# yuvalH9/UMERegRobust

Hardware: AMD Instinct MI355X
Metric: registration_pairs_per_s (higher is better)
Workload: dtype f32

## Files before the change

umeregrobust_amd/csrc/match_dev.h:

```cpp
#pragma once
#include "common.h"
#include "qlayout.h"

namespace umereg {

using f32x16 = __attribute__((ext_vector_type(16))) float;
using half8 = __attribute__((ext_vector_type(8))) _Float16;
using f32x2 = __attribute__((ext_vector_type(2))) float;

constexpr int kDistWaves = 4;

constexpr int kRegionCap = 512;
constexpr int kMaxSplits = 64;
constexpr unsigned int kShareMask = 0x8000808bu;

struct MatchScratch {
    unsigned int* rowlim;
    unsigned int* cnt;
    unsigned int* cand;
    int splits;
    unsigned int share_mask;
    int force_exhaustive;
    const int* ord1;
    const int* ord2;
    unsigned long long* stats;
};

constexpr int kCoarseTA = 2;
constexpr int kCoarseRows = kCoarseTA * 8;
constexpr int kCoarseWG = kCoarseRows * kDistWaves;

constexpr int kPK = 33;
constexpr int kPWaves = 8;
constexpr int kPRows = 32;
constexpr int kPWG = kPRows * kPWaves;
constexpr int kPRegionCap = 1024;

inline size_t qa_bytes(int n1) { return align_up((size_t)n1, 128) * 128 * sizeof(float); }
inline size_t qb_bytes(int n2) { return align_up((size_t)n2, 32) * 128 * sizeof(float); }
struct CoarsePlan {
    int n_ablk, n_blocks, n_btiles, splits, tiles_per_split;
    int sub_tiles, sub_tps, sub_splits;
};
struct MatchOpts {
    int variant = 0;
    int splits = 0;
    long long share_mask = -1;
    int exhaustive = 0;
};
inline int resolve_opts(const umereg_match_opts* o, MatchOpts& m, const char* who)
{
    m = MatchOpts();
    if (!o) return UMEREG_OK;
    UMEREG_REQUIRE(o->variant == 0 || o->variant == 1, "%s: unknown matcher variant %d (0 = Q-form, 1 = P-form)", who, (int)o->variant);
    UMEREG_REQUIRE(o->splits >= 0 && o->force_exhaustive >= 0, "%s: negative matcher option", who);
    UMEREG_REQUIRE(o->share_mask <= 0xffffffffll, "%s: share_mask does not fit 32 bits", who);
    UMEREG_REQUIRE(o->reserved == 0, "%s: umereg_match_opts.reserved must be 0 (got %d)", who, (int)o->reserved);
    m.variant = o->variant;
    m.splits = o->splits;
    m.share_mask = o->share_mask;
    m.exhaustive = o->force_exhaustive ? 1 : 0;
    return UMEREG_OK;
}
inline bool use_pform(const MatchOpts& o) { return o.variant == 1; }
constexpr int kNumCU = 256;
#ifndef UMEREG_COARSE_PHASES
#define UMEREG_COARSE_PHASES 3
#endif
constexpr int kMinSplitTiles = 4;
constexpr int kLeadMinTiles = 64;

inline CoarsePlan coarse_plan(int n1, int n2, const MatchOpts& o)
{
    CoarsePlan p;
    p.n_btiles = (n2 + 31) / 32;
    int splits;
    if (use_pform(o)) {
        p.n_ablk = (n1 + kPWG - 1) / kPWG;
        p.n_blocks = p.n_ablk * kPWaves;
        splits = kNumCU / p.n_ablk;
    } else {
        p.n_ablk = (n1 + kCoarseWG - 1) / kCoarseWG;
        p.n_blocks = p.n_ablk * kDistWaves;
        splits = (2560 + p.n_ablk - 1) / p.n_ablk;
    }
    p.sub_tiles = p.sub_tps = p.sub_splits = 0;
    if (UMEREG_COARSE_PHASES >= 2 && !use_pform(o) && o.splits <= 0 && p.n_btiles >= kLeadMinTiles) {
        const int n_sub = (n2 + kSubStride - 1) / kSubStride;
        p.sub_tiles = (n_sub + 31) / 32;
        int s1 = 4 * kNumCU / p.n_ablk;
        s1 = s1 < 1 ? 1 : (s1 > 16 ? 16 : s1);
        s1 = s1 > p.sub_tiles / kMinSplitTiles ? p.sub_tiles / kMinSplitTiles : s1;
        p.sub_tps = (p.sub_tiles + s1 - 1) / s1;
        p.sub_splits = (p.sub_tiles + p.sub_tps - 1) / p.sub_tps;
        const int bulk = p.n_btiles - p.sub_tiles;
        int s2 = splits > kMaxSplits - 16 ? kMaxSplits - 16 : splits;
        s2 = s2 > bulk / kMinSplitTiles ? bulk / kMinSplitTiles : s2;
        p.tiles_per_split = (bulk + s2 - 1) / s2;
        p.splits = p.sub_splits + (bulk + p.tiles_per_split - 1) / p.tiles_per_split;
        return p;
    }
    if (o.splits > 0) splits = o.splits;
    if (splits > kMaxSplits) splits = kMaxSplits;
    if (splits > p.n_btiles) splits = p.n_btiles;
    if (splits < 1) splits = 1;
    p.tiles_per_split = (p.n_btiles + splits - 1) / splits;
    p.splits = (p.n_btiles + p.tiles_per_split - 1) / p.tiles_per_split;
    return p;
}
inline size_t region_cap(const MatchOpts& o) { return use_pform(o) ? (size_t)kPRegionCap : (size_t)kRegionCap; }
inline size_t cand_bytes(int n1, const CoarsePlan& p, const MatchOpts& o)
{
    return align_up(((size_t)n1 + (size_t)p.n_blocks * p.splits * (1 + region_cap(o))) * sizeof(unsigned int), 256);
}
inline size_t pfrag_bytes(const CoarsePlan& p, const MatchOpts& o)
{
    return use_pform(o) ? ((size_t)p.n_blocks + (size_t)p.n_btiles) * kPK * 64 * sizeof(half8) : 0;
}
#ifndef UMEREG_COARSE_STATS
#define UMEREG_COARSE_STATS 0
#endif
constexpr size_t kStatsBytes = UMEREG_COARSE_STATS ? 256 : 0;
inline size_t match_scratch_bytes(int n1, int n2, const MatchOpts& o = MatchOpts())
{
    const CoarsePlan p = coarse_plan(n1, n2, o);
    return cand_bytes(n1, p, o) + pfrag_bytes(p, o) + kStatsBytes;
}

inline int match_args(const void* Q1_rows_h, const void* Q2_cols_h, int n1, int n2, void* scratch, size_t scratch_bytes,
                      const MatchOpts& o, const char* who)
{
    UMEREG_REQUIRE(Q1_rows_h && Q2_cols_h, "%s: null basis pointer", who);
// ... 40 lines not shown
```

umeregrobust_amd/csrc/match_f16r.hip:

```cpp
#include <type_traits>

#include "common.h"
#include "match_dev.h"
#include "qlayout.h"

namespace umereg {

constexpr float kCoarseMargin = 0.03125f + 0.0009765625f;
constexpr float kCoarseTermMax = 1.00390625f;
#ifndef UMEREG_COARSE_EXIT
#define UMEREG_COARSE_EXIT 3
#endif

__device__ __forceinline__ float group32_max(float v)
{
    int x = __float_as_int(v);
    x = __float_as_int(fmaxf(__int_as_float(x), __int_as_float(__builtin_amdgcn_mov_dpp(x, 0xB1, 0xf, 0xf, true))));
    x = __float_as_int(fmaxf(__int_as_float(x), __int_as_float(__builtin_amdgcn_mov_dpp(x, 0x4E, 0xf, 0xf, true))));
    x = __float_as_int(fmaxf(__int_as_float(x), __int_as_float(__builtin_amdgcn_mov_dpp(x, 0x141, 0xf, 0xf, true))));
    x = __float_as_int(fmaxf(__int_as_float(x), __int_as_float(__builtin_amdgcn_mov_dpp(x, 0x140, 0xf, 0xf, true))));
    x = __float_as_int(fmaxf(__int_as_float(x), __int_as_float(__builtin_amdgcn_ds_swizzle(x, 0x401F))));
    return __int_as_float(x);
}

#ifndef UMEREG_COARSE_ABLATE
#define UMEREG_COARSE_ABLATE 0
#endif
#ifndef UMEREG_COARSE_TPS
#define UMEREG_COARSE_TPS 2
#endif
constexpr int kCoarseTPS = UMEREG_COARSE_TPS;

__global__ __launch_bounds__(kWave* kDistWaves, 2) void ume_coarse_h_kernel(
    const half8* __restrict__ Afrag, const half8* __restrict__ Bfrag, int n1, int n2, int n_ablk, int tile_lo, int tile_mid, int tile_hi,
    int lead_tps, int lead_splits, int tiles_per_split, int sp0, MatchScratch ms)
{
    __shared__ half8 ldsB[2][kCoarseTPS * 512];
    const int wave = __builtin_amdgcn_readfirstlane(threadIdx.x >> 6);
    const int lane = lane_id();
    const int ablk = blockIdx.x % n_ablk;
    const int spl = blockIdx.x / n_ablk;
    const int sp = sp0 + spl;
    const bool lead = spl < lead_splits;
    const int jt0 = lead ? tile_lo + spl * lead_tps : tile_mid + (spl - lead_splits) * tiles_per_split;
    const int jt1 = lead ? min(jt0 + lead_tps, tile_mid) : min(jt0 + tiles_per_split, tile_hi);
    const int h = lane >> 5;
    const int i_base = ablk * kCoarseWG + wave * kCoarseRows;

    half8 a[kCoarseTA][2];
#pragma unroll
    for (int t = 0; t < kCoarseTA; ++t)
#pragma unroll
        for (int s = 0; s < 2; ++s)
            a[t][s] = Afrag[((((size_t)(ablk * (kCoarseWG / 8) + wave * kCoarseTA + t)) * 2 + s) * 2 + 0) * 64 + lane];

    int lim[kCoarseTA][4];
    unsigned int seen[kCoarseTA][4];
#pragma unroll
    for (int t = 0; t < kCoarseTA; ++t)
#pragma unroll
        for (int g = 0; g < 4; ++g) {
            const int i = i_base + t * 8 + 2 * g + h;
            seen[t][g] = __hip_atomic_load(ms.rowlim + min(i, n1 - 1), __ATOMIC_RELAXED, __HIP_MEMORY_SCOPE_AGENT);
            lim[t][g] = i < n1 ? max(__float_as_int(1.0e-30f), (int)seen[t][g]) : __float_as_int(3.0e38f);
        }
#pragma unroll
    for (int t = 0; t < kCoarseTA; ++t)
#pragma unroll
        for (int s = 0; s < 2; ++s) asm volatile("" ::"v"(a[t][s]));

    const int blk = ablk * kDistWaves + wave;
    unsigned int* const region = ms.cand + ((size_t)blk * ms.splits + sp) * kRegionCap;
    int qn = 0;
    auto share = [&](bool reload) __attribute__((always_inline)) {
#pragma unroll
        for (int t = 0; t < kCoarseTA; ++t)
#pragma unroll
            for (int g = 0; g < 4; ++g) {
                const float v = group32_max(__int_as_float(lim[t][g]));
                const int i = i_base + t * 8 + 2 * g + h;
                if ((lane & 31) == 0 && i < n1 && __float_as_uint(v) > seen[t][g]) atomicMax(ms.rowlim + i, __float_as_uint(v));
                lim[t][g] = max(__float_as_int(v), (int)seen[t][g]);
            }
        if (reload) {
#pragma unroll
            for (int t = 0; t < kCoarseTA; ++t)
#pragma unroll
                for (int g = 0; g < 4; ++g) {
                    const int i = min(i_base + t * 8 + 2 * g + h, n1 - 1);
                    seen[t][g] = __hip_atomic_load(ms.rowlim + i, __ATOMIC_RELAXED, __HIP_MEMORY_SCOPE_AGENT);
                }
        }
    };

    half8 st[kCoarseTPS][2];
    const int c0 = threadIdx.x, c1 = 256 + threadIdx.x;
    const int src0 = ((c0 >> 6) * 2) * 64 + (c0 & 63), src1 = ((c1 >> 6) * 2) * 64 + (c1 & 63);
    auto gload = [&](int jg) __attribute__((always_inline)) {
#pragma unroll
        for (int q = 0; q < kCoarseTPS; ++q) {
            const int jt = min(jg + q, jt1 - 1);
            st[q][0] = Bfrag[(size_t)jt * 1024 + src0];
            st[q][1] = Bfrag[(size_t)jt * 1024 + src1];
        }
    };
    auto lstore = [&](int buf) __attribute__((always_inline)) {
#pragma unroll
        for (int q = 0; q < kCoarseTPS; ++q) {
            ldsB[buf][q * 512 + c0] = st[q][0];
            ldsB[buf][q * 512 + c1] = st[q][1];
        }
    };
    if (jt0 < jt1) {
        gload(jt0);
        lstore(0);
    }
    if (jt0 + kCoarseTPS < jt1) gload(jt0 + kCoarseTPS);
    __syncthreads();
    int cur = 0;
    auto share_point = [&](const int jt) __attribute__((always_inline)) {
        const int kt = jt - jt0;
        if ((ms.share_mask >> (kt < 31 ? kt : 31)) & 1u) {
            if (kt < 31 || (kt & 31) == 31) share(true);
        }
    };
#if UMEREG_COARSE_STATS
    unsigned int n_stop1 = 0, n_stop2 = 0;
#endif
    auto hopeless = [&](const float (&sc)[kCoarseTA][4], const int cols) __attribute__((always_inline)) {
        float d = sc[0][0] - __int_as_float(lim[0][0]);
#pragma unroll
        for (int t = 0; t < kCoarseTA; ++t)
#pragma unroll
            for (int g = 0; g < 4; ++g) d = fmaxf(d, sc[t][g] - __int_as_float(lim[t][g]));
        const bool stop = __builtin_amdgcn_ballot_w64(!(d < -(float)(4 - cols) * kCoarseTermMax)) == 0ull;
        return (UMEREG_COARSE_ABLATE & 16) ? true : stop;
    };
    auto filter = [&](const int jt, const float (&sc)[kCoarseTA][4]) __attribute__((always_inline)) {
        if (UMEREG_COARSE_ABLATE & 2) {
#pragma unroll
            for (int t = 0; t < kCoarseTA; ++t)
#pragma unroll
                for (int g = 0; g < 4; ++g) lim[t][g] = max(lim[t][g], __float_as_int(sc[t][g]));
            return;
        }
#pragma unroll
        for (int t = 0; t < kCoarseTA; ++t)
#pragma unroll
            for (int g = 0; g < 4; ++g) lim[t][g] = max(lim[t][g], __float_as_int(sc[t][g] - kCoarseMargin));
        share_point(jt);
        unsigned long long hit[kCoarseTA][4], any = 0;
// ... 8 lines not shown
#pragma unroll
            for (int t = 0; t < kCoarseTA; ++t)
#pragma unroll
                for (int g = 0; g < 4; ++g) lim[t][g] = __float_as_int(group32_max(__int_as_float(lim[t][g])));
            any = 0;
#pragma unroll
            for (int t = 0; t < kCoarseTA; ++t)
#pragma unroll
                for (int g = 0; g < 4; ++g) {
                    hit[t][g] = __builtin_amdgcn_ballot_w64(sc[t][g] >= __int_as_float(lim[t][g]));
                    any |= hit[t][g];
                }
        }
        if (any) {
            const unsigned int j = (unsigned int)(jt * 32 + (lane & 31));
#pragma unroll
            for (int t = 0; t < kCoarseTA; ++t)
#pragma unroll
                for (int g = 0; g < 4; ++g) {
                    const unsigned long long mask = hit[t][g];
                    if (mask) {
                        const int pos = qn + mbcnt(mask);
                        if (((mask >> lane) & 1ull) && pos < kRegionCap)
                            region[pos] = ((unsigned int)(t * 8 + 2 * g + h) << 27) | j;
                        qn += __builtin_popcountll(mask);
                    }
                }
        }
    };
    auto tile = [&](const int jt, const int q) __attribute__((always_inline)) {
        const half8* const lB = &ldsB[cur][q * 512];
        float sc[kCoarseTA][4];
        auto products = [&](const int b, f32x16 (&cc)[kCoarseTA]) __attribute__((always_inline)) {
            const half8 b0 = (UMEREG_COARSE_ABLATE & 8) ? a[0][0] : lB[(b * 2 + 0) * 64 + lane];
            const half8 b1 = (UMEREG_COARSE_ABLATE & 8) ? a[0][1] : lB[(b * 2 + 1) * 64 + lane];
            if (UMEREG_COARSE_ABLATE & 4) {
#pragma unroll
                for (int t = 0; t < kCoarseTA; ++t)
#pragma unroll
                    for (int e = 0; e < 16; ++e) cc[t][e] = (float)b0[e & 7] + (float)b1[(e + t) & 7];
            } else {
#pragma unroll
                for (int t = 0; t < kCoarseTA; ++t) cc[t] = __builtin_amdgcn_mfma_f32_32x32x16_f16(a[t][0], b0, f32x16{0}, 0, 0, 0);
#pragma unroll
                for (int t = 0; t < kCoarseTA; ++t) cc[t] = __builtin_amdgcn_mfma_f32_32x32x16_f16(a[t][1], b1, cc[t], 0, 0, 0);
            }
        };
        auto squares = [&](const int b, const f32x16 (&cc)[kCoarseTA]) __attribute__((always_inline)) {
#pragma unroll
            for (int t = 0; t < kCoarseTA; ++t)
#pragma unroll
                for (int g = 0; g < 4; ++g) {
                    if (UMEREG_COARSE_ABLATE & 1) {
                        sc[t][g] = b == 0 ? cc[t][4 * g] : sc[t][g] + cc[t][4 * g + 1];
                        continue;
                    }
                    float acc = b == 0 ? cc[t][4 * g] * cc[t][4 * g] : fmaf(cc[t][4 * g], cc[t][4 * g], sc[t][g]);
                    acc = fmaf(cc[t][4 * g + 1], cc[t][4 * g + 1], acc);
                    acc = fmaf(cc[t][4 * g + 2], cc[t][4 * g + 2], acc);
                    sc[t][g] = fmaf(cc[t][4 * g + 3], cc[t][4 * g + 3], acc);
                }
        };
        constexpr bool kTest1 = (UMEREG_COARSE_EXIT & 1) && !(UMEREG_COARSE_ABLATE & 15), kTest2 = (UMEREG_COARSE_EXIT & 2) && !(UMEREG_COARSE_ABLATE & 15);
        constexpr bool kAhead = (UMEREG_COARSE_EXIT & 4) != 0;
        f32x16 c0[kCoarseTA], c1[kCoarseTA];
        products(0, c0);
        if (kAhead || !kTest1) products(1, c1);
        squares(0, c0);
        if (kTest1 && hopeless(sc, 1)) {
#if UMEREG_COARSE_STATS
            ++n_stop1;
#endif
            share_point(jt);
            return;
        }
        if (!kAhead && kTest1) products(1, c1);
        squares(1, c1);
        if (kTest2 && hopeless(sc, 2)) {
#if UMEREG_COARSE_STATS
            ++n_stop2;
#endif
            share_point(jt);
            return;
        }
#pragma unroll
        for (int b = 2; b < 4; ++b) {
            f32x16 cc[kCoarseTA];
            products(b, cc);
            squares(b, cc);
        }
        filter(jt, sc);
    };
    for (int jg = jt0; jg < jt1; jg += kCoarseTPS) {
#pragma unroll
        for (int q = 0; q < kCoarseTPS; ++q)
            if (jg + q < jt1) tile(jg + q, q);
        if (jg + kCoarseTPS < jt1) lstore(cur ^ 1);
        if (jg + 2 * kCoarseTPS < jt1) gload(jg + 2 * kCoarseTPS);
        __syncthreads();
        cur ^= 1;
    }
    share(false);
    if (lane == 0) ms.cnt[(size_t)blk * ms.splits + sp] = (unsigned int)qn;
#if UMEREG_COARSE_STATS
    if (lane == 0) {
        atomicAdd(ms.stats + 0, (unsigned long long)max(jt1 - jt0, 0));
        atomicAdd(ms.stats + 1, (unsigned long long)n_stop1);
        atomicAdd(ms.stats + 2, (unsigned long long)n_stop2);
        atomicAdd(ms.stats + 3, (unsigned long long)qn);
    }
#endif
}

constexpr float kCoarseMarginP = 0.009765625f;
constexpr int kPDepth = 5;
constexpr int kQsStride = 33;

__global__ __launch_bounds__(256) void pform_pack_kernel(const _Float16* __restrict__ Ah, const _Float16* __restrict__ Bh, int n1,
                                                         int n2, int tiles1, int tiles2, half8* __restrict__ PA,
                                                         half8* __restrict__ PB)
{
    __shared__ float4 qs[32 * kQsStride];
    const int side = blockIdx.y, tile = blockIdx.x;
    if (tile >= (side ? tiles2 : tiles1)) return;
    const int n = side ? n2 : n1;
    const _Float16* const Q = side ? Bh : Ah;
    half8* const P = (side ? PB : PA) + (size_t)tile * kPK * 64;
    const int tid = threadIdx.x;
    if (tile * 32 >= n) {
        for (int o = tid; o < kPK * 64; o += 256) P[o] = half8{0};
        return;
// ... 396 lines not shown
```

umeregrobust_amd/csrc/ball_moment.hip:

```cpp
#include "grid.h"

namespace umereg {

constexpr int kPackWG = 1024;
constexpr int kPackMaxBlocks = 32;

__global__ __launch_bounds__(kPackWG) void pack_points_kernel(const float* __restrict__ pts, char* __restrict__ ws,
                                                              size_t ws_stride, int N, const PairDesc* __restrict__ desc)
{
    __shared__ unsigned int red[kPackWG / 64][6];
    const GridWs w = grid_ws(N);
    const int b = blockIdx.y;
    const int n_live = desc ? desc->n_pts[b] : N;
    const UMEREG_GLOBAL_AS float* __restrict__ src = global_ptr(desc ? desc->pts[b] : pts + (size_t)b * N * 3);
    float4* out = reinterpret_cast<float4*>(ws + b * ws_stride + w.off_p4o);
    unsigned int* bbox = reinterpret_cast<unsigned int*>(ws + b * ws_stride + w.off_bbox);
    unsigned int e[6] = {0u, 0u, 0u, 0u, 0u, 0u};
    for (int j = blockIdx.x * kPackWG + threadIdx.x; j < w.Npad; j += gridDim.x * kPackWG) {
        float4 v = make_float4(kFar, kFar, kFar, 0.f);
        if (j < n_live) {
            const UMEREG_GLOBAL_AS float* p = src + (size_t)j * 3;
            v = make_float4(p[0], p[1], p[2], 0.f);
            const unsigned int ex = enc_ord(v.x), ey = enc_ord(v.y), ez = enc_ord(v.z);
            e[0] = max(e[0], ~ex); e[1] = max(e[1], ~ey); e[2] = max(e[2], ~ez);
// ... 297 lines not shown
                                                const Grid& g, float qx, float qy, float qz, float r2, int K,
                                                int n_eff, int nbits, int* lst, int cap, int lane)
{
    const float rq = sqrtf(r2) * 1.0001f + 1e-20f;
    const int y0 = cell_axis(qy - rq, g.miny, g.invy, g.ny), y1 = cell_axis(qy + rq, g.miny, g.invy, g.ny);
    const int z0 = cell_axis(qz - rq, g.minz, g.invz, g.nz), z1 = cell_axis(qz + rq, g.minz, g.invz, g.nz);
    const float csy = 1.0f / g.invy, csz = 1.0f / g.invz;
    const float rq2 = rq * rq;
    int cnt = 0;
    int thr = n_eff - 1;
    const int ny_r = y1 - y0 + 1, n_rows = ny_r * (z1 - z0 + 1);
    for (int r0 = 0; r0 < n_rows; r0 += kWave) {
        int my_beg = 0, my_end = 0;
        {
            const int r = r0 + lane;
            const int z = z0 + r / ny_r, y = y0 + r % ny_r;
            const float z_a = g.minz + (float)z * csz, z_b = z_a + csz;
            const float dzc = fmaxf(fmaxf(z > 0 ? z_a - qz : 0.f, z < g.nz - 1 ? qz - z_b : 0.f), 0.f) * 0.9999f;
            const float y_a = g.miny + (float)y * csy, y_b = y_a + csy;
            const float dyc = fmaxf(fmaxf(y > 0 ? y_a - qy : 0.f, y < g.ny - 1 ? qy - y_b : 0.f), 0.f) * 0.9999f;
            const float rem = rq2 - dyc * dyc - dzc * dzc;
            if (r < n_rows && rem > 0.f) {
                const float sx = sqrtf(rem) * 1.0001f + 1e-20f;
                const int cbase = (z * g.ny + y) * g.nx;
                my_beg = start[cbase + cell_axis(qx - sx, g.minx, g.invx, g.nx)];
                my_end = start[cbase + cell_axis(qx + sx, g.minx, g.invx, g.nx) + 1];
            }
        }
        const int n_here = min(kWave, n_rows - r0);
        for (int rr = 0; rr < n_here; ++rr) {
            const int beg = __builtin_amdgcn_readlane(my_beg, rr);
            const int end = __builtin_amdgcn_readlane(my_end, rr);
            if (beg >= end) continue;
            auto scan = [&](int base, auto U_) __attribute__((always_inline)) {
                constexpr int U = decltype(U_)::value;
                float4 pv[U];
#pragma unroll
                for (int u = 0; u < U; ++u) {
                    const int pos = base + u * kWave + lane;
                    pv[u] = P4s[pos < end ? pos : end - 1];
                }
#pragma unroll
                for (int u = 0; u < U; ++u) {
                    const int pos = base + u * kWave + lane;
                    const float4 p = pv[u];
                    const int oi = __float_as_int(p.w);
                    const float dx = qx - p.x;
                    const float dy = qy - p.y;
                    const float dz = qz - p.z;
                    const float d2 = dist2_as_the_reference<kFma>(dx, dy, dz);
                    const bool hit = (pos < end) && (d2 < r2) && (oi <= thr);
                    const unsigned long long m = __ballot(hit);
                    if (m != 0ull) {
                        if (hit) lst[cnt + mbcnt(m)] = oi;
                        cnt += __popcll(m);
                    }
                }
            };
            auto make_room = [&](int chunks) __attribute__((always_inline)) {
                if (cnt > cap - chunks * kWave) {
                    __builtin_amdgcn_wave_barrier();
                    cnt = keep_k_smallest(lst, cnt, K, nbits, cap, lane, thr);
                }
            };
            int base = beg;
            for (; end - base > 2 * kWave; base += kWave * kScanUnroll) { make_room(kScanUnroll); scan(base, std::integral_constant<int, kScanUnroll>{}); }
            if (base < end) { make_room(2); scan(base, std::integral_constant<int, 2>{}); }
        }
    }
    __builtin_amdgcn_wave_barrier();
    if (cnt > K) cnt = keep_k_smallest(lst, cnt, K, nbits, cap, lane, thr);
    return cnt;
}

__device__ __forceinline__ void bitonic_sort(int* lst, int n_pow2, int lane)
{
    for (int k = 2; k <= n_pow2; k <<= 1)
        for (int j = k >> 1; j > 0; j >>= 1) {
            __builtin_amdgcn_wave_barrier();
            for (int t = lane; t < (n_pow2 >> 1); t += kWave) {
                const int lo = ((t & ~(j - 1)) << 1) | (t & (j - 1));
                const int hi = lo | j;
                const bool up = (lo & k) == 0;
                const int a = lst[lo], b = lst[hi];
                if ((a > b) == up) { lst[lo] = b; lst[hi] = a; }
            }
        }
    __builtin_amdgcn_wave_barrier();
}

__device__ __forceinline__ void sort_kept(int* lst, int count, int lane)
{
    int n_pow2 = 64;
    while (n_pow2 < count) n_pow2 <<= 1;
    for (int e = count + lane; e < n_pow2; e += kWave) lst[e] = 0x7fffffff;
    bitonic_sort(lst, n_pow2, lane);
}

template <bool kFma>
__global__ __launch_bounds__(256) void ball_query_kernel(
// ... 86 lines not shown
    for (int k = threadIdx.x + kKeep * 1024; k < n_kp; k += 1024) atomicAdd(&cnt[cell_of_kp(k)], 1);
    __syncthreads();
    const int c0 = threadIdx.x * 4;
    const int t0 = cnt[c0], t1 = cnt[c0 + 1], t2 = cnt[c0 + 2], t3 = cnt[c0 + 3];
    const int sum = t0 + t1 + t2 + t3;
    int incl = sum;
#pragma unroll
    for (int m = 1; m < 64; m <<= 1) {
        const int o = __shfl_up(incl, m, kWave);
        if ((int)(threadIdx.x & 63) >= m) incl += o;
    }
    if ((threadIdx.x & 63) == 63) part[threadIdx.x >> 6] = incl;
    __syncthreads();
    int base = 0;
    for (int k = 0; k < (int)(threadIdx.x >> 6); ++k) base += part[k];
    const int excl = base + incl - sum;
    __syncthreads();
    cnt[c0] = excl; cnt[c0 + 1] = excl + t0; cnt[c0 + 2] = excl + t0 + t1; cnt[c0 + 3] = excl + t0 + t1 + t2;
    __syncthreads();
#pragma unroll
    for (int u = 0; u < kKeep; ++u)
        if (mine[u] >= 0) perm[atomicAdd(&cnt[mine[u]], 1)] = threadIdx.x + u * 1024;
    for (int k = threadIdx.x + kKeep * 1024; k < n_kp; k += 1024) perm[atomicAdd(&cnt[cell_of_kp(k)], 1)] = k;
}

__device__ __forceinline__ float bcast8(float v)
{
    int x = __float_as_int(v);
    x = __builtin_amdgcn_mov_dpp(x, 0x00, 0xf, 0xf, true);
    x = __builtin_amdgcn_update_dpp(x, x, 0x114, 0xf, 0xa, false);
    return __int_as_float(x);
}

constexpr int kMomUnroll = 4;

template <int kAcc, bool kFma = false, bool kDesc = false>
__global__ __launch_bounds__(256) void ume_moments_kernel(
    const char* __restrict__ ws, size_t ws_stride, const float* __restrict__ kpts,
    const int64_t* __restrict__ kp_index, const float4* __restrict__ feat4, int N, int n_kp, int K, int cap,
    float radius, int flags, float* __restrict__ F, int32_t* __restrict__ nn_count,
    int64_t* __restrict__ nn_idx)
{
    const bool ordered = flags & UMEREG_MOMENTS_ORDERED;
    extern __shared__ int lds[];
    const int wave = __builtin_amdgcn_readfirstlane(threadIdx.x >> 6);
    const int lane = lane_id();
    const int b = blockIdx.y;
    const GridWs w = grid_ws(N);
    const char* wb = ws + b * ws_stride;
    int kp;
    if (ordered) {
        const int nblk = gridDim.x, xcd = blockIdx.x & 7, q = nblk >> 3, r = nblk & 7;
        const int lblk = (xcd < r ? xcd * (q + 1) : r * (q + 1) + (xcd - r) * q) + (blockIdx.x >> 3);
        const int slot = lblk * (blockDim.x >> 6) + wave;
        if (slot >= n_kp) return;
        kp = __builtin_amdgcn_readfirstlane(reinterpret_cast<const int*>(wb + w.off_kperm)[slot]);
    } else {
        kp = blockIdx.x * (blockDim.x >> 6) + wave;
        if (kp >= n_kp) return;
    }
    int* lst = lds + wave * cap;
    const float4* Pb = reinterpret_cast<const float4*>(wb + w.off_p4o);
    const float4* P4s = reinterpret_cast<const float4*>(wb + w.off_p4s);
    const int* start = reinterpret_cast<const int*>(wb + w.off_start);
    const Grid g = load_grid(reinterpret_cast<const unsigned int*>(wb + w.off_bbox), radius, N);
    const unsigned int* __restrict__ rec = reinterpret_cast<const unsigned int*>(wb + w.off_bbox);
// ... 9 lines not shown
            for (int e = lane; e < 128; e += kWave) F[((size_t)b * n_kp + kp) * 128 + e] = __int_as_float(0x7fc00000);
            if (nn_count && lane == 0) nn_count[(size_t)b * n_kp + kp] = 0;
            if (nn_idx) for (int e = lane; e < K; e += kWave) nn_idx[((size_t)b * n_kp + kp) * K + e] = -1;
            return;
        }
        const float4 qp = Pb[ki];
        qx = qp.x; qy = qp.y; qz = qp.z;
    } else {
        const float* q = kpts + ((size_t)b * n_kp + kp) * 3;
        qx = q[0]; qy = q[1]; qz = q[2];
    }
    const int nbits = 32 - __clz(N > 1 ? N - 1 : 1);

    const int count = ball_search_grid<kFma>(P4s, start, g, qx, qy, qz, radius * radius, K, n_live, nbits, lst, cap, lane);

    if (nn_count && lane == 0) nn_count[(size_t)b * n_kp + kp] = count;
    if (nn_idx) {
        sort_kept(lst, count, lane);
        int64_t* o = nn_idx + ((size_t)b * n_kp + kp) * K;
        for (int e = lane; e < K; e += kWave) o[e] = e < count ? (int64_t)lst[e] : (int64_t)-1;
    }

    constexpr bool kF64 = kAcc != 0;
#ifndef UMEREG_MOM_ABLATE
#define UMEREG_MOM_ABLATE 0
#endif
#ifndef UMEREG_MOM_MFMA_UNROLL
#define UMEREG_MOM_MFMA_UNROLL 4
#endif
    if (kAcc == 2) {
        constexpr int kMU = UMEREG_MOM_MFMA_UNROLL;
        const int mk = lane >> 4, mr = lane & 15, mcq = mr & 7, mns = 4 * (mr >> 3) + mk, mj = lane & 3;
        const float* Pf = reinterpret_cast<const float*>(Pb);
        double acc[4] = {0.0, 0.0, 0.0, 0.0};
        auto mtrip = [&](int e0, bool ragged, auto U_) __attribute__((always_inline)) {
            constexpr int kU = decltype(U_)::value;
            float4 ff[kU];
            float pc[kU];
#pragma unroll
            for (int u = 0; u < kU; ++u) {
                const unsigned int jn = (unsigned int)lst[min(e0 + u * 8 + mns, count - 1)];
                if (UMEREG_MOM_ABLATE & 2) {
                    const float v = __uint_as_float(0x3f800000u | (jn & 0xffffu));
                    ff[u] = make_float4(v, v + 1.f, v + 2.f, v + 3.f);
                    pc[u] = v;
                    continue;
                }
                ff[u] = feat_slice((size_t)jn * 8 + mcq);
                pc[u] = Pf[(size_t)jn * 4 + (mj > 0 ? mj - 1 : 0)];
            }
            if (UMEREG_MOM_ABLATE & 4) {
                float t = 0.f;
#pragma unroll
                for (int u = 0; u < kU; ++u) t += ((ff[u].x + ff[u].y) + (ff[u].z + ff[u].w)) + pc[u];
                acc[0] += (double)t;
                return;
            }
#pragma unroll
            for (int u = 0; u < kU; ++u) {
                if (ragged) {
                    const bool v = e0 + u * 8 + mns < count;
                    ff[u].x = v ? ff[u].x : 0.f; ff[u].y = v ? ff[u].y : 0.f;
                    ff[u].z = v ? ff[u].z : 0.f; ff[u].w = v ? ff[u].w : 0.f;
                }
                const double bq = mj == 0 ? 1.0 : (double)pc[u];
                acc[0] = __builtin_amdgcn_mfma_f64_4x4x4f64((double)ff[u].x, bq, acc[0], 0, 0, 0);
                acc[1] = __builtin_amdgcn_mfma_f64_4x4x4f64((double)ff[u].y, bq, acc[1], 0, 0, 0);
                acc[2] = __builtin_amdgcn_mfma_f64_4x4x4f64((double)ff[u].z, bq, acc[2], 0, 0, 0);
                acc[3] = __builtin_amdgcn_mfma_f64_4x4x4f64((double)ff[u].w, bq, acc[3], 0, 0, 0);
            }
        };
#ifndef UMEREG_MOM_PIPE
#define UMEREG_MOM_PIPE 0
#endif
#if UMEREG_MOM_PIPE
        constexpr int kH = kMU / 2 > 0 ? kMU / 2 : 1;
        auto load_half = [&](int e0, float4 (&ff)[kH], float (&pc)[kH]) __attribute__((always_inline)) {
#pragma unroll
            for (int u = 0; u < kH; ++u) {
                if (e0 + u * 8 < count) {
                    const unsigned int jn = (unsigned int)lst[min(e0 + u * 8 + mns, count - 1)];
                    ff[u] = feat_slice((size_t)jn * 8 + mcq);
                    pc[u] = Pf[(size_t)jn * 4 + (mj > 0 ? mj - 1 : 0)];
                }
            }
        };
        auto fma_half = [&](int e0, float4 (&ff)[kH], float (&pc)[kH]) __attribute__((always_inline)) {
#pragma unroll
            for (int u = 0; u < kH; ++u) {
                if (e0 + u * 8 < count) {
                    if (e0 + u * 8 + 8 > count) {
                        const bool v = e0 + u * 8 + mns < count;
                        ff[u].x = v ? ff[u].x : 0.f; ff[u].y = v ? ff[u].y : 0.f;
                        ff[u].z = v ? ff[u].z : 0.f; ff[u].w = v ? ff[u].w : 0.f;
                    }
                    const double bq = mj == 0 ? 1.0 : (double)pc[u];
                    acc[0] = __builtin_amdgcn_mfma_f64_4x4x4f64((double)ff[u].x, bq, acc[0], 0, 0, 0);
                    acc[1] = __builtin_amdgcn_mfma_f64_4x4x4f64((double)ff[u].y, bq, acc[1], 0, 0, 0);
                    acc[2] = __builtin_amdgcn_mfma_f64_4x4x4f64((double)ff[u].z, bq, acc[2], 0, 0, 0);
                    acc[3] = __builtin_amdgcn_mfma_f64_4x4x4f64((double)ff[u].w, bq, acc[3], 0, 0, 0);
                }
            }
        };
        {
            float4 fa[kH], fc[kH];
            float pa[kH], pq[kH];
            const int step = 8 * kH;
            const int n_half = (UMEREG_MOM_ABLATE & 1) ? 0 : (count + step - 1) / step;
            if (n_half > 0) load_half(0, fa, pa);
            for (int h = 0; h < n_half; h += 2) {
                if (h + 1 < n_half) load_half((h + 1) * step, fc, pq);
                fma_half(h * step, fa, pa);
                if (h + 2 < n_half) load_half((h + 2) * step, fa, pa);
                if (h + 1 < n_half) fma_half((h + 1) * step, fc, pq);
            }
        }
        (void)mtrip;
#else
        const int mfull = (UMEREG_MOM_ABLATE & 1) ? 0 : (count / (8 * kMU)) * (8 * kMU);
        for (int e0 = 0; e0 < mfull; e0 += 8 * kMU) mtrip(e0, false, std::integral_constant<int, kMU>{});
        if (!(UMEREG_MOM_ABLATE & 1))
        for (int e0 = mfull; e0 < count; e0 += 8) mtrip(e0, e0 + 8 > count, std::integral_constant<int, 1>{});
#endif
#pragma unroll
        for (int m = 0; m < 4; ++m) acc[m] += shfl_xor_f64(acc[m], 8);
        const bool lower = (lane & 8) == 0;
        double s = (lower && mj == 0) ? (acc[0] + acc[1]) + (acc[2] + acc[3]) : 0.0;
#pragma unroll
        for (int m = 1; m < 64; m <<= 1) s += shfl_xor_f64(s, m);
// ... 217 lines not shown
    UMEREG_REQUIRE(pts && packed, "pack_points: null pointer");
    UMEREG_REQUIRE(B > 0 && N > 0, "pack_points: B, N must be positive (got %d, %d)", B, N);
    UMEREG_REQUIRE(radius > 0.f, "pack_points: radius must be positive");
    if (int rc = check_device()) return rc;
    if (packed_bytes < umereg_ume_moments_workspace_bytes(B, N) || ((uintptr_t)packed & 15)) {
        set_error("pack_points: packed buffer too small or misaligned (%zu < %zu)", packed_bytes,
                  umereg_ume_moments_workspace_bytes(B, N));
        return UMEREG_EWORKSPACE;
    }
    return launch_prep(pts, (char*)packed, B, N, radius, (hipStream_t)stream);
}

UMEREG_API int umereg_ume_keypoint_order(void* packed, const float* kpts, const int64_t* kp_index, int B, int N,
                                         int n_kp, float radius, void* stream)
{
    UMEREG_REQUIRE(packed && (kpts || kp_index), "keypoint_order: null pointer");
    UMEREG_REQUIRE(B > 0 && N > 0 && n_kp > 0, "keypoint_order: B, N, n_kp must be positive");
    UMEREG_REQUIRE(n_kp <= grid_ws(N).Npad, "keypoint_order: n_kp (%d) exceeds the order buffer (%d)", n_kp, grid_ws(N).Npad);
    if (int rc = check_device()) return rc;
    hipLaunchKernelGGL(kp_order_kernel, dim3(1, B), dim3(1024), 0, (hipStream_t)stream, (char*)packed, grid_ws(N).total,
                       kpts, kp_index, N, n_kp, radius, (const PairDesc*)nullptr);
    UMEREG_CHECK_LAUNCH("kp_order_kernel");
    return UMEREG_OK;
}

namespace umereg {
int launch_moments(const void* packed, const float* kpts, const int64_t* kp_index, const float* feat, int B, int N, int n_kp, int K,
                   float radius, int flags, float* F, int32_t* nn_count, int64_t* nn_idx, hipStream_t st, const PairDesc* desc)
{
    int cap, waves;
    lds_plan(K, &cap, &waves);
    dim3 grid((n_kp + waves - 1) / waves, B);
    UMEREG_REQUIRE(!((flags & UMEREG_MOMENTS_ACC_F32) && (flags & UMEREG_MOMENTS_ACC_VALU)), "ume_moments: ACC_F32 and ACC_VALU exclude each other");
    UMEREG_REQUIRE(!((flags & UMEREG_MOMENTS_FMA_DIST) && (flags & (UMEREG_MOMENTS_ACC_F32 | UMEREG_MOMENTS_ACC_VALU))),
                   "ume_moments: FMA_DIST goes with the default accumulation only");
#define UMEREG_LAUNCH_MOMENTS(...)                                                                                                    \
    hipLaunchKernelGGL((ume_moments_kernel<__VA_ARGS__>), grid, dim3(kWave * waves), (size_t)waves * cap * sizeof(int), st,               \
                       (const char*)packed, grid_ws(N).total, kpts, kp_index, (const float4*)feat, N, n_kp, K, cap, radius, flags, F,   \
                       nn_count, nn_idx)
    UMEREG_REQUIRE(!desc || !(flags & (UMEREG_MOMENTS_FMA_DIST | UMEREG_MOMENTS_ACC_F32 | UMEREG_MOMENTS_ACC_VALU)),
                   "ume_moments: a ragged pair runs the default kernel only");
    if (desc)
        UMEREG_LAUNCH_MOMENTS(2, false, true);
    else if (flags & UMEREG_MOMENTS_FMA_DIST)
        UMEREG_LAUNCH_MOMENTS(2, true);
    else if (!(flags & (UMEREG_MOMENTS_ACC_F32 | UMEREG_MOMENTS_ACC_VALU)))
        UMEREG_LAUNCH_MOMENTS(2);
    else if (!(flags & UMEREG_MOMENTS_ACC_F32))
        UMEREG_LAUNCH_MOMENTS(1);
    else
        UMEREG_LAUNCH_MOMENTS(0);
#undef UMEREG_LAUNCH_MOMENTS
    UMEREG_CHECK_LAUNCH("ume_moments_kernel");
    return UMEREG_OK;
}
}

UMEREG_API int umereg_ume_moments_packed_f32(const void* packed, const float* kpts, const int64_t* kp_index,
                                             const float* feat, int B, int N, int n_kp, int feat_dim, int K,
                                             float radius, int flags, float* F, int32_t* nn_count, int64_t* nn_idx,
                                             void* stream)
{
    UMEREG_REQUIRE(packed && (kpts || kp_index) && feat && F, "ume_moments: null pointer (packed/kpts|kp_index/feat/F)");
    UMEREG_REQUIRE(feat_dim == UMEREG_FEAT_DIM,
                   "ume_moments: feature dim must be 32 like the reference (evaluate.py:55), got %d", feat_dim);
    UMEREG_REQUIRE(B > 0 && N > 0 && n_kp > 0, "ume_moments: B, N, n_kp must be positive (got %d, %d, %d)", B, N, n_kp);
// ... 27 lines not shown
```

Baseline: 3875.

## Stage coarse-match B tiles directly into LDS and raise occupancy bound

The coarse matcher kernel now loads B-fragment tiles straight from global memory into LDS with global_load_lds, prefetching the next tile group into the alternate buffer. This removes the register staging copies and the separate LDS store step. Row limits are likewise fetched asynchronously into a small LDS array instead of per-lane registers. Launch bounds are raised from 2 to 4 resident workgroups per CU, and the planner merges a tiny trailing split into the previous one. The costs are explicit vmcnt/lgkmcnt waits, inline-asm LDS reads that may serialize MFMA issue, and a tighter register budget that could cause spills.

```diff
diff --git a/umeregrobust_amd/csrc/match_dev.h b/umeregrobust_amd/csrc/match_dev.h
--- a/umeregrobust_amd/csrc/match_dev.h
+++ b/umeregrobust_amd/csrc/match_dev.h
@@ -29,6 +29,7 @@
 constexpr int kCoarseTA = 2;
 constexpr int kCoarseRows = kCoarseTA * 8;
 constexpr int kCoarseWG = kCoarseRows * kDistWaves;
+constexpr int kCoarseResidentPerCU = 4;
 
 constexpr int kPK = 33;
 constexpr int kPWaves = 8;
@@ -88,7 +89,7 @@
     if (UMEREG_COARSE_PHASES >= 2 && !use_pform(o) && o.splits <= 0 && p.n_btiles >= kLeadMinTiles) {
         const int n_sub = (n2 + kSubStride - 1) / kSubStride;
         p.sub_tiles = (n_sub + 31) / 32;
-        int s1 = 4 * kNumCU / p.n_ablk;
+        int s1 = kCoarseResidentPerCU * kNumCU / p.n_ablk;
         s1 = s1 < 1 ? 1 : (s1 > 16 ? 16 : s1);
         s1 = s1 > p.sub_tiles / kMinSplitTiles ? p.sub_tiles / kMinSplitTiles : s1;
         p.sub_tps = (p.sub_tiles + s1 - 1) / s1;
@@ -97,7 +98,9 @@
         int s2 = splits > kMaxSplits - 16 ? kMaxSplits - 16 : splits;
         s2 = s2 > bulk / kMinSplitTiles ? bulk / kMinSplitTiles : s2;
         p.tiles_per_split = (bulk + s2 - 1) / s2;
-        p.splits = p.sub_splits + (bulk + p.tiles_per_split - 1) / p.tiles_per_split;
+        int n_bulk = (bulk + p.tiles_per_split - 1) / p.tiles_per_split;
+        if (n_bulk > 1 && bulk - (n_bulk - 1) * p.tiles_per_split < kMinSplitTiles) --n_bulk;
+        p.splits = p.sub_splits + n_bulk;
         return p;
     }
     if (o.splits > 0) splits = o.splits;
diff --git a/umeregrobust_amd/csrc/match_f16r.hip b/umeregrobust_amd/csrc/match_f16r.hip
--- a/umeregrobust_amd/csrc/match_f16r.hip
+++ b/umeregrobust_amd/csrc/match_f16r.hip
@@ -31,11 +31,15 @@
 #endif
 constexpr int kCoarseTPS = UMEREG_COARSE_TPS;
 
-__global__ __launch_bounds__(kWave* kDistWaves, 2) void ume_coarse_h_kernel(
+#ifndef UMEREG_COARSE_DIRECT
+#define UMEREG_COARSE_DIRECT 1
+#endif
+__global__ __launch_bounds__(kWave* kDistWaves, kCoarseResidentPerCU) void ume_coarse_h_kernel(
     const half8* __restrict__ Afrag, const half8* __restrict__ Bfrag, int n1, int n2, int n_ablk, int tile_lo, int tile_mid, int tile_hi,
     int lead_tps, int lead_splits, int tiles_per_split, int sp0, MatchScratch ms)
 {
     __shared__ half8 ldsB[2][kCoarseTPS * 512];
+    __shared__ __attribute__((aligned(16))) unsigned int seenL[kDistWaves][kCoarseRows];
     const int wave = __builtin_amdgcn_readfirstlane(threadIdx.x >> 6);
     const int lane = lane_id();
     const int ablk = blockIdx.x % n_ablk;
@@ -43,7 +47,7 @@
     const int sp = sp0 + spl;
     const bool lead = spl < lead_splits;
     const int jt0 = lead ? tile_lo + spl * lead_tps : tile_mid + (spl - lead_splits) * tiles_per_split;
-    const int jt1 = lead ? min(jt0 + lead_tps, tile_mid) : min(jt0 + tiles_per_split, tile_hi);
+    const int jt1 = lead ? min(jt0 + lead_tps, tile_mid) : (sp == ms.splits - 1 ? tile_hi : min(jt0 + tiles_per_split, tile_hi));
     const int h = lane >> 5;
     const int i_base = ablk * kCoarseWG + wave * kCoarseRows;
 
@@ -55,15 +59,11 @@
             a[t][s] = Afrag[((((size_t)(ablk * (kCoarseWG / 8) + wave * kCoarseTA + t)) * 2 + s) * 2 + 0) * 64 + lane];
 
     int lim[kCoarseTA][4];
-    unsigned int seen[kCoarseTA][4];
-#pragma unroll
-    for (int t = 0; t < kCoarseTA; ++t)
-#pragma unroll
-        for (int g = 0; g < 4; ++g) {
-            const int i = i_base + t * 8 + 2 * g + h;
-            seen[t][g] = __hip_atomic_load(ms.rowlim + min(i, n1 - 1), __ATOMIC_RELAXED, __HIP_MEMORY_SCOPE_AGENT);
-            lim[t][g] = i < n1 ? max(__float_as_int(1.0e-30f), (int)seen[t][g]) : __float_as_int(3.0e38f);
-        }
+    auto fetch_seen = [&]() __attribute__((always_inline)) {
+        if (lane < kCoarseRows)
+            __builtin_amdgcn_global_load_lds((const __attribute__((address_space(1))) void*)(ms.rowlim + min(i_base + lane, n1 - 1)),
+                                             (__attribute__((address_space(3))) void*)(&seenL[wave][0]), 4, 0, 16 );
+    };
 #pragma unroll
     for (int t = 0; t < kCoarseTA; ++t)
 #pragma unroll
@@ -73,32 +73,37 @@
     unsigned int* const region = ms.cand + ((size_t)blk * ms.splits + sp) * kRegionCap;
     int qn = 0;
     auto share = [&](bool reload) __attribute__((always_inline)) {
+        asm volatile("s_waitcnt vmcnt(0)" ::: "memory");
 #pragma unroll
         for (int t = 0; t < kCoarseTA; ++t)
 #pragma unroll
             for (int g = 0; g < 4; ++g) {
                 const float v = group32_max(__int_as_float(lim[t][g]));
-                const int i = i_base + t * 8 + 2 * g + h;
-                if ((lane & 31) == 0 && i < n1 && __float_as_uint(v) > seen[t][g]) atomicMax(ms.rowlim + i, __float_as_uint(v));
-                lim[t][g] = max(__float_as_int(v), (int)seen[t][g]);
-            }
-        if (reload) {
-#pragma unroll
-            for (int t = 0; t < kCoarseTA; ++t)
-#pragma unroll
-                for (int g = 0; g < 4; ++g) {
-                    const int i = min(i_base + t * 8 + 2 * g + h, n1 - 1);
-                    seen[t][g] = __hip_atomic_load(ms.rowlim + i, __ATOMIC_RELAXED, __HIP_MEMORY_SCOPE_AGENT);
-                }
-        }
-    };
-
-    half8 st[kCoarseTPS][2];
+                const int r = t * 8 + 2 * g + h;
+                const unsigned int seen = seenL[wave][r];
+                if ((lane & 31) == 0 && i_base + r < n1 && __float_as_uint(v) > seen) atomicMax(ms.rowlim + i_base + r, __float_as_uint(v));
+                lim[t][g] = max(__float_as_int(v), (int)seen);
+            }
+        if (reload) fetch_seen();
+    };
+
+    constexpr bool kDirect = UMEREG_COARSE_DIRECT != 0;
+    half8 st[kDirect ? 1 : kCoarseTPS][2];
     const int c0 = threadIdx.x, c1 = 256 + threadIdx.x;
     const int src0 = ((c0 >> 6) * 2) * 64 + (c0 & 63), src1 = ((c1 >> 6) * 2) * 64 + (c1 & 63);
+    auto stage = [&](int jg, int buf) __attribute__((always_inline)) {
+#pragma unroll
+        for (int q = 0; q < kCoarseTPS; ++q) {
+            const half8* const src = Bfrag + (size_t)min(jg + q, jt1 - 1) * 1024 + lane;
+#pragma unroll
+            for (int r = 0; r < 2; ++r)
+                __builtin_amdgcn_global_load_lds((const __attribute__((address_space(1))) void*)(src + ((r * 4 + wave) * 2) * 64),
+                                                 (__attribute__((address_space(3))) void*)(&ldsB[buf][q * 512 + r * 256 + wave * 64]), 16, 0, 0);
+        }
+    };
     auto gload = [&](int jg) __attribute__((always_inline)) {
 #pragma unroll
-        for (int q = 0; q < kCoarseTPS; ++q) {
+        for (int q = 0; q < (kDirect ? 0 : kCoarseTPS); ++q) {
             const int jt = min(jg + q, jt1 - 1);
             st[q][0] = Bfrag[(size_t)jt * 1024 + src0];
             st[q][1] = Bfrag[(size_t)jt * 1024 + src1];
@@ -106,17 +111,32 @@
     };
     auto lstore = [&](int buf) __attribute__((always_inline)) {
 #pragma unroll
-        for (int q = 0; q < kCoarseTPS; ++q) {
+        for (int q = 0; q < (kDirect ? 0 : kCoarseTPS); ++q) {
             ldsB[buf][q * 512 + c0] = st[q][0];
             ldsB[buf][q * 512 + c1] = st[q][1];
         }
     };
-    if (jt0 < jt1) {
-        gload(jt0);
-        lstore(0);
-    }
-    if (jt0 + kCoarseTPS < jt1) gload(jt0 + kCoarseTPS);
+    fetch_seen();
+    if (kDirect) {
+        if (jt0 < jt1) stage(jt0, 0);
+        asm volatile("s_waitcnt vmcnt(0)" ::: "memory");
+    } else {
+        if (jt0 < jt1) {
+            gload(jt0);
+            lstore(0);
+        }
+        asm volatile("s_waitcnt vmcnt(0)" ::: "memory");
+        if (jt0 + kCoarseTPS < jt1) gload(jt0 + kCoarseTPS);
+    }
     __syncthreads();
+#pragma unroll
+    for (int t = 0; t < kCoarseTA; ++t)
+#pragma unroll
+        for (int g = 0; g < 4; ++g) {
+            const int r = t * 8 + 2 * g + h;
+            const int seen = (int)seenL[wave][r];
+            lim[t][g] = i_base + r < n1 ? max(__float_as_int(1.0e-30f), seen) : __float_as_int(3.0e38f);
+        }
     int cur = 0;
     auto share_point = [&](const int jt) __attribute__((always_inline)) {
         const int kt = jt - jt0;
@@ -191,8 +211,20 @@
         const half8* const lB = &ldsB[cur][q * 512];
         float sc[kCoarseTA][4];
         auto products = [&](const int b, f32x16 (&cc)[kCoarseTA]) __attribute__((always_inline)) {
-            const half8 b0 = (UMEREG_COARSE_ABLATE & 8) ? a[0][0] : lB[(b * 2 + 0) * 64 + lane];
-            const half8 b1 = (UMEREG_COARSE_ABLATE & 8) ? a[0][1] : lB[(b * 2 + 1) * 64 + lane];
+            half8 b0, b1;
+            if (UMEREG_COARSE_ABLATE & 8) {
+                b0 = a[0][0];
+                b1 = a[0][1];
+            } else if (kDirect) {
+                const unsigned int addr = (unsigned int)(size_t)(const __attribute__((address_space(3))) half8*)(lB + lane);
+                asm volatile("ds_read_b128 %0, %2 offset:%3\n\tds_read_b128 %1, %2 offset:%4\n\ts_waitcnt lgkmcnt(0)"
+                             : "=&v"(b0), "=&v"(b1)
+                             : "v"(addr), "n"((b * 2 + 0) * 1024), "n"((b * 2 + 1) * 1024)
+                             : "memory");
+            } else {
+                b0 = lB[(b * 2 + 0) * 64 + lane];
+                b1 = lB[(b * 2 + 1) * 64 + lane];
+            }
             if (UMEREG_COARSE_ABLATE & 4) {
 #pragma unroll
                 for (int t = 0; t < kCoarseTA; ++t)
@@ -251,11 +283,16 @@
         filter(jt, sc);
     };
     for (int jg = jt0; jg < jt1; jg += kCoarseTPS) {
+        if (kDirect && jg + kCoarseTPS < jt1) stage(jg + kCoarseTPS, cur ^ 1);
 #pragma unroll
         for (int q = 0; q < kCoarseTPS; ++q)
             if (jg + q < jt1) tile(jg + q, q);
-        if (jg + kCoarseTPS < jt1) lstore(cur ^ 1);
-        if (jg + 2 * kCoarseTPS < jt1) gload(jg + 2 * kCoarseTPS);
+        if (kDirect) {
+            asm volatile("s_waitcnt vmcnt(0)" ::: "memory");
+        } else {
+            if (jg + kCoarseTPS < jt1) lstore(cur ^ 1);
+            if (jg + 2 * kCoarseTPS < jt1) gload(jg + 2 * kCoarseTPS);
+        }
         __syncthreads();
         cur ^= 1;
     }
```

After: 4137, median of 5. +6.8%, better.

## Specialize ball-scan tail chunks and use 32-bit offsets in moment gathers

Applied to the files above, without the earlier changes.

The neighbour scan loop now picks among 1-4 chunk variants at compile time. Only the final chunk of a tail trip clamps its index, and a precomputed live mask replaces the per-lane bounds test. The hit ballot is split into two ballots and lanes test membership with inverse_ballot. In the MFMA moment gather, feature and coordinate loads switch to 32-bit byte offsets from a global base, and the list index is clamped only on ragged trips. This is meant to cut address arithmetic and VGPR pressure, at the cost of a new N <= 2^25 limit and more code size.

```diff
diff --git a/umeregrobust_amd/csrc/ball_moment.hip b/umeregrobust_amd/csrc/ball_moment.hip
--- a/umeregrobust_amd/csrc/ball_moment.hip
+++ b/umeregrobust_amd/csrc/ball_moment.hip
@@ -353,40 +353,47 @@
             const int beg = __builtin_amdgcn_readlane(my_beg, rr);
             const int end = __builtin_amdgcn_readlane(my_end, rr);
             if (beg >= end) continue;
-            auto scan = [&](int base, auto U_) __attribute__((always_inline)) {
-                constexpr int U = decltype(U_)::value;
-                float4 pv[U];
-#pragma unroll
-                for (int u = 0; u < U; ++u) {
-                    const int pos = base + u * kWave + lane;
-                    pv[u] = P4s[pos < end ? pos : end - 1];
+            auto scan = [&](int base, auto C_, auto kTail_) __attribute__((always_inline)) {
+                constexpr int C = decltype(C_)::value;
+                constexpr bool kTail = decltype(kTail_)::value;
+                typedef float f4v __attribute__((ext_vector_type(4)));
+                const f4v* __restrict__ P = reinterpret_cast<const f4v*>(P4s);
+                f4v pv[C];
+#pragma unroll
+                for (int u = 0; u < C; ++u) {
+                    int pos = base + u * kWave + lane;
+                    if (kTail && u == C - 1) pos = min(pos, end - 1);
+                    pv[u] = P[pos];
                 }
-#pragma unroll
-                for (int u = 0; u < U; ++u) {
-                    const int pos = base + u * kWave + lane;
-                    const float4 p = pv[u];
+                const unsigned long long live = kTail ? ~0ull >> (C * kWave - (end - base)) : ~0ull;
+#pragma unroll
+                for (int u = 0; u < C; ++u) {
+                    const f4v p = pv[u];
                     const int oi = __float_as_int(p.w);
                     const float dx = qx - p.x;
                     const float dy = qy - p.y;
                     const float dz = qz - p.z;
                     const float d2 = dist2_as_the_reference<kFma>(dx, dy, dz);
-                    const bool hit = (pos < end) && (d2 < r2) && (oi <= thr);
-                    const unsigned long long m = __ballot(hit);
-                    if (m != 0ull) {
-                        if (hit) lst[cnt + mbcnt(m)] = oi;
-                        cnt += __popcll(m);
-                    }
+                    unsigned long long m = __ballot(d2 < r2) & __ballot(oi <= thr);
+                    if (kTail && u == C - 1) m &= live;
+                    if (__builtin_amdgcn_inverse_ballot_w64(m)) lst[cnt + mbcnt(m)] = oi;
+                    cnt += __popcll(m);
                 }
             };
-            auto make_room = [&](int chunks) __attribute__((always_inline)) {
-                if (cnt > cap - chunks * kWave) {
+            static_assert(kScanUnroll == 4, "the tail forms are written out for trips of up to 4 chunks");
+            for (int base = beg; base < end; base += kWave * kScanUnroll) {
+                const int left = end - base;
+                const int c = left >= kScanUnroll * kWave ? kScanUnroll : (left + kWave - 1) / kWave;
+                if (cnt > cap - c * kWave) {
                     __builtin_amdgcn_wave_barrier();
                     cnt = keep_k_smallest(lst, cnt, K, nbits, cap, lane, thr);
                 }
-            };
-            int base = beg;
-            for (; end - base > 2 * kWave; base += kWave * kScanUnroll) { make_room(kScanUnroll); scan(base, std::integral_constant<int, kScanUnroll>{}); }
-            if (base < end) { make_room(2); scan(base, std::integral_constant<int, 2>{}); }
+                if (left >= kScanUnroll * kWave) scan(base, std::integral_constant<int, 4>{}, std::false_type{});
+                else if (c == 1) scan(base, std::integral_constant<int, 1>{}, std::true_type{});
+                else if (c == 2) scan(base, std::integral_constant<int, 2>{}, std::true_type{});
+                else if (c == 3) scan(base, std::integral_constant<int, 3>{}, std::true_type{});
+                else scan(base, std::integral_constant<int, 4>{}, std::true_type{});
+            }
         }
     }
     __builtin_amdgcn_wave_barrier();
@@ -539,6 +546,9 @@
     return __int_as_float(x);
 }
 
+#ifndef UMEREG_MOM_OFF32
+#define UMEREG_MOM_OFF32 1
+#endif
 constexpr int kMomUnroll = 4;
 
 template <int kAcc, bool kFma = false, bool kDesc = false>
@@ -614,22 +624,42 @@
         constexpr int kMU = UMEREG_MOM_MFMA_UNROLL;
         const int mk = lane >> 4, mr = lane & 15, mcq = mr & 7, mns = 4 * (mr >> 3) + mk, mj = lane & 3;
         const float* Pf = reinterpret_cast<const float*>(Pb);
+        const UMEREG_GLOBAL_AS char* Pg = reinterpret_cast<const UMEREG_GLOBAL_AS char*>(global_ptr(Pf));
+        const UMEREG_GLOBAL_AS char* fg = reinterpret_cast<const UMEREG_GLOBAL_AS char*>(fb);
+        auto feat_at = [&](unsigned int off) __attribute__((always_inline)) {
+            const f4v t = *reinterpret_cast<const UMEREG_GLOBAL_AS f4v*>(fg + off);
+            return make_float4(t.x, t.y, t.z, t.w);
+        };
+        auto coord_at = [&](unsigned int off) __attribute__((always_inline)) { return *reinterpret_cast<const UMEREG_GLOBAL_AS float*>(Pg + off); };
+        (void)Pf; (void)feat_at; (void)coord_at;
         double acc[4] = {0.0, 0.0, 0.0, 0.0};
+        auto one_or = [&](float c) __attribute__((always_inline)) {
+            float v = mj == 0 ? 1.0f : c;
+            asm("" : "+v"(v));
+            return v;
+        };
         auto mtrip = [&](int e0, bool ragged, auto U_) __attribute__((always_inline)) {
             constexpr int kU = decltype(U_)::value;
             float4 ff[kU];
             float pc[kU];
+            unsigned int jn[kU];
+#pragma unroll
+            for (int u = 0; u < kU; ++u) jn[u] = (unsigned int)lst[ragged ? min(e0 + u * 8 + mns, count - 1) : e0 + u * 8 + mns];
 #pragma unroll
             for (int u = 0; u < kU; ++u) {
-                const unsigned int jn = (unsigned int)lst[min(e0 + u * 8 + mns, count - 1)];
                 if (UMEREG_MOM_ABLATE & 2) {
-                    const float v = __uint_as_float(0x3f800000u | (jn & 0xffffu));
+                    const float v = __uint_as_float(0x3f800000u | (jn[u] & 0xffffu));
                     ff[u] = make_float4(v, v + 1.f, v + 2.f, v + 3.f);
                     pc[u] = v;
                     continue;
                 }
-                ff[u] = feat_slice((size_t)jn * 8 + mcq);
-                pc[u] = Pf[(size_t)jn * 4 + (mj > 0 ? mj - 1 : 0)];
+#if UMEREG_MOM_OFF32
+                ff[u] = feat_at(jn[u] * 128u + (unsigned int)mcq * 16u);
+                pc[u] = coord_at(jn[u] * 16u + (unsigned int)(mj > 0 ? mj - 1 : 0) * 4u);
+#else
+                ff[u] = feat_slice((size_t)jn[u] * 8 + mcq);
+                pc[u] = Pf[(size_t)jn[u] * 4 + (mj > 0 ? mj - 1 : 0)];
+#endif
             }
             if (UMEREG_MOM_ABLATE & 4) {
                 float t = 0.f;
@@ -645,7 +675,7 @@
                     ff[u].x = v ? ff[u].x : 0.f; ff[u].y = v ? ff[u].y : 0.f;
                     ff[u].z = v ? ff[u].z : 0.f; ff[u].w = v ? ff[u].w : 0.f;
                 }
-                const double bq = mj == 0 ? 1.0 : (double)pc[u];
+                const double bq = (double)one_or(pc[u]);
                 acc[0] = __builtin_amdgcn_mfma_f64_4x4x4f64((double)ff[u].x, bq, acc[0], 0, 0, 0);
                 acc[1] = __builtin_amdgcn_mfma_f64_4x4x4f64((double)ff[u].y, bq, acc[1], 0, 0, 0);
                 acc[2] = __builtin_amdgcn_mfma_f64_4x4x4f64((double)ff[u].z, bq, acc[2], 0, 0, 0);
@@ -676,7 +706,7 @@
                         ff[u].x = v ? ff[u].x : 0.f; ff[u].y = v ? ff[u].y : 0.f;
                         ff[u].z = v ? ff[u].z : 0.f; ff[u].w = v ? ff[u].w : 0.f;
                     }
-                    const double bq = mj == 0 ? 1.0 : (double)pc[u];
+                    const double bq = (double)one_or(pc[u]);
                     acc[0] = __builtin_amdgcn_mfma_f64_4x4x4f64((double)ff[u].x, bq, acc[0], 0, 0, 0);
                     acc[1] = __builtin_amdgcn_mfma_f64_4x4x4f64((double)ff[u].y, bq, acc[1], 0, 0, 0);
                     acc[2] = __builtin_amdgcn_mfma_f64_4x4x4f64((double)ff[u].z, bq, acc[2], 0, 0, 0);
@@ -960,6 +990,7 @@
     lds_plan(K, &cap, &waves);
     dim3 grid((n_kp + waves - 1) / waves, B);
     UMEREG_REQUIRE(!((flags & UMEREG_MOMENTS_ACC_F32) && (flags & UMEREG_MOMENTS_ACC_VALU)), "ume_moments: ACC_F32 and ACC_VALU exclude each other");
+    UMEREG_REQUIRE(!UMEREG_MOM_OFF32 || N <= (1 << 25), "ume_moments: N must be <= 2^25 (32-bit byte offsets into the feature table), got %d", N);
     UMEREG_REQUIRE(!((flags & UMEREG_MOMENTS_FMA_DIST) && (flags & (UMEREG_MOMENTS_ACC_F32 | UMEREG_MOMENTS_ACC_VALU))),
                    "ume_moments: FMA_DIST goes with the default accumulation only");
 #define UMEREG_LAUNCH_MOMENTS(...)                                                                                                    \
```

Measured after the change: 3953 before, 3740 after. 0.946x the previous value.
